# MIT-SPARK/Khronos

Hardware: AMD Instinct MI355X
Metric: active-window frames/sec (+ Mvoxel-updates/sec) at 1280x720 RGB-D+labels, 2 cm voxels (higher is better)
Workload: dtype f32

## Files before the change

### khronos_amd/csrc/khr_device.h

```cpp
#pragma once
#include <hip/hip_runtime.h>
#include <stdint.h>

namespace khr {

constexpr uint64_t kEmptyKey = ~0ull;
constexpr uint32_t kInvalidSlot = 0xffffffffu;

constexpr uint32_t BLK_UPDATED = 1u, BLK_MESH_UPDATED = 2u, BLK_TRACKING_UPDATED = 4u, BLK_HAS_ACTIVE = 8u,
                   BLK_LIVE = 16u,
                   BLK_TRACK_DIRTY = 32u,
                   BLK_ANY_KEEP = 64u,
                   BLK_HAS_NEG = 128u;
constexpr uint8_t VOX_ACTIVE = 1, VOX_EVER_FREE = 2, VOX_TO_REMOVE = 4, VOX_SEM_VALID = 8;
constexpr uint8_t VOX_OCC = 16;
constexpr uint8_t VOX_PUBLIC_MASK = 0x0f;

enum Counter : int {
  C_FREE_HEAD = 0,
  C_N_FREE,
  C_MAX_SLOT,
  C_N_VISIBLE,
  C_N_NEW,
  C_N_EF,
  C_N_LIVE,
  C_POOL_EXHAUSTED,
  C_N_UPD_LO,
  C_N_REMOVED,
  C_N_SEEDS,
  C_N_MESH,
  C_N_BAND,
  C_N_TSDF,
  C_BAND_OVERFLOW,
  C_TSDF_CURSOR,
  C_MESH_OVERFLOW,
  C_N_PROC,
  C_N_EF_A,
  C_N_PROC2,
  C_N_EF2,
  C_MP_DONE,
  C_N_ITEMS0,
  C_N_ITEMS1,
  C_N_ITEMS2,
  C_N_ITEMS3,
  C_COUNT = 32
};
enum Stat64 : int { S_UPD = 0 , S_BAND , S_MESH_VERTS, S_PRUNED, S_CUM_UPD, S_CUM_BAND, S_CUM_VISITED, S_CUM_CALLS, S_COUNT = 8 };

struct MeshDesc {
  uint32_t offset;
  uint32_t count;
};

struct DevMap {
  uint64_t* ht_keys;
  uint32_t* ht_vals;
  uint32_t ht_mask;
  uint32_t capacity;
  int4* blk_index;
  uint32_t* blk_flags;
  float* dist;
  float* weight;
  uint32_t* color;
  uint64_t* last_obs;
  ulonglong2* obs;
  uint64_t* last_occ;
  uint64_t* trk_lim;
  uint8_t* vflags;
  uint32_t* sem_label;
  float* lik;
  uint64_t* freebits;
  uint16_t* blk_band;
  uint32_t* free_slots;
  uint32_t* counters;
  unsigned long long* stats;
  MeshDesc* mesh_desc;
};

constexpr int kBandSlots = 32;
constexpr uint16_t kItemTouched = 0x8000u, kItemNeg = 0x4000u, kItemBandMask = 0x3fffu;
struct FuseList {
  uint4* a;
  uint4* b;
  uint32_t cap;
  uint32_t* counts;
};
__device__ inline uint32_t fuseClass(uint32_t band) { return band > 128u ? 0u : (band > 64u ? 1u : (band > 0u ? 2u : 3u)); }
__device__ inline uint4* fuseDescPtr(const FuseList& l, uint32_t cls, uint32_t pos) {
  uint4* const arr = cls < 2u ? l.a : l.b;
  return arr + ((cls & 1u) ? l.cap - 1u - pos : pos);
}

__host__ __device__ inline int likStride(int K) { return K <= 4 ? K : ((K + 31) & ~31); }

struct DevParams {
  float vs, vs_inv, bs, bs_inv, trunc;
  int vps, nvox, K;
  int KS;
  int with_semantics, with_tracking;
  int use_dropoff, const_weight, interp, range_mode, sem_mode;
  float dropoff_eps, max_weight, adaptive_diff, log_match, log_nomatch;
  float occ_thr;
  double temporal_buffer, temporal_window;
  int nn;
  float mesh_min_weight;
  float mesh_eps;
  int mesh_attr_source;
  int alloc_candidate;
  int rank, world;
  int dbg;
};

struct DevFrame {
  const float* depth;
  const float* range;
  const uint32_t* rgba;
  const int32_t* label;
  int32_t* dyn;
  const int32_t* obj;
  int W, H;
  float fx, fy, cx, cy, min_range, max_range;
  float R[9], t[3];
  float Rw[9], tw[3];
  uint64_t stamp;
  int has_color, has_label;
};

struct DevFrustum {
  float n[4][3];
  float infl;
  int3 bc;
  int n_steps;
  int max_steps;
  float tw[3];
};

__host__ __device__ inline uint32_t mix32(uint32_t h) {
  h ^= h >> 16;
  h *= 0x85ebca6bu;
  h ^= h >> 13;
  h *= 0xc2b2ae35u;
  h ^= h >> 16;
  return h;
}

__host__ __device__ inline int ownerOf(int x, int y, int z, int world) {
  if (world <= 1) return 0;
  const uint32_t h = mix32(static_cast<uint32_t>(x) * 73856093u ^
                           mix32(static_cast<uint32_t>(y) * 19349663u ^ mix32(static_cast<uint32_t>(z) * 83492791u)));
  return static_cast<int>((static_cast<uint64_t>(h) * static_cast<uint64_t>(world)) >> 32);
}

__host__ __device__ inline uint64_t packKey(int x, int y, int z) {
  return (static_cast<uint64_t>(static_cast<uint32_t>(x + (1 << 20)) & 0x1fffffu)) |
         (static_cast<uint64_t>(static_cast<uint32_t>(y + (1 << 20)) & 0x1fffffu) << 21) |
         (static_cast<uint64_t>(static_cast<uint32_t>(z + (1 << 20)) & 0x1fffffu) << 42);
}
__host__ __device__ inline void unpackKey(uint64_t k, int* x, int* y, int* z) {
  *x = static_cast<int>(k & 0x1fffffu) - (1 << 20);
  *y = static_cast<int>((k >> 21) & 0x1fffffu) - (1 << 20);
  *z = static_cast<int>((k >> 42) & 0x1fffffu) - (1 << 20);
}
__host__ __device__ inline uint32_t hashKey(uint64_t k) {
  return mix32(static_cast<uint32_t>(k) ^ mix32(static_cast<uint32_t>(k >> 32) + 0x9e3779b9u));
}

__device__ inline uint32_t htLookup(const DevMap& m, uint64_t key) {
  uint32_t h = hashKey(key) & m.ht_mask;
  while (true) {
    const uint64_t k = m.ht_keys[h];
    if (k == key) return m.ht_vals[h];
    if (k == kEmptyKey) return kInvalidSlot;
    h = (h + 1) & m.ht_mask;
  }
}

__device__ inline void htInsertUnique(const DevMap& m, uint64_t key, uint32_t slot) {
  uint32_t h = hashKey(key) & m.ht_mask;
  while (true) {
    const unsigned long long prev =
        atomicCAS(reinterpret_cast<unsigned long long*>(&m.ht_keys[h]), static_cast<unsigned long long>(kEmptyKey),
                  static_cast<unsigned long long>(key));
    if (prev == kEmptyKey) {
      m.ht_vals[h] = slot;
      return;
    }
    h = (h + 1) & m.ht_mask;
  }
}

__device__ inline void xform(const float* R, const float* t, float x, float y, float z, float* o) {
  o[0] = ((R[0] * x + R[1] * y) + R[2] * z) + t[0];
  o[1] = ((R[3] * x + R[4] * y) + R[5] * z) + t[1];
  o[2] = ((R[6] * x + R[7] * y) + R[8] * z) + t[2];
}

__device__ inline bool pointInFrustum(const DevFrustum& fr, const float* pc, float max_range) {
  bool in = !(pc[2] < -fr.infl);
  const float n2 = (pc[0] * pc[0] + pc[1] * pc[1]) + pc[2] * pc[2];
  const float lim = max_range + fr.infl;
  in = in && !(n2 > lim * lim);
#pragma unroll
  for (int k = 0; k < 4; ++k) {
    const float d = (pc[0] * fr.n[k][0] + pc[1] * fr.n[k][1]) + pc[2] * fr.n[k][2];
    in = in && !(d < -fr.infl);
  }
  return in;
}
__device__ inline bool blockIsCandidate(const DevParams& p, const DevFrustum& fr, const float* R, const float* t, float max_range,
                                        int bx, int by, int bz) {
  if (p.alloc_candidate == 0) {
    float pc[3];
    xform(R, t, (static_cast<float>(bx) + 0.5f) * p.bs, (static_cast<float>(by) + 0.5f) * p.bs, (static_cast<float>(bz) + 0.5f) * p.bs, pc);
    return pointInFrustum(fr, pc, max_range);
  }
  const int b[3] = {bx, by, bz}, bc[3] = {fr.bc.x, fr.bc.y, fr.bc.z};
  float cand[3][2];
  int nc[3];
#pragma unroll
  for (int a = 0; a < 3; ++a) {
    nc[a] = 0;
#pragma unroll
    for (int e = -1; e <= 1; ++e) {
      const int d = b[a] - bc[a] + e;
      if (d < -fr.max_steps || d > fr.max_steps) continue;
      const float pw = fr.tw[a] + static_cast<float>(d) * p.bs;
      if (static_cast<int>(floorf(pw * p.bs_inv)) == b[a] && nc[a] < 2) cand[a][nc[a]++] = pw;
    }
  }
  for (int i = 0; i < nc[0]; ++i)
    for (int j = 0; j < nc[1]; ++j)
      for (int k = 0; k < nc[2]; ++k) {
        float pc[3];
        xform(R, t, cand[0][i], cand[1][j], cand[2][k], pc);
        if (pointInFrustum(fr, pc, max_range)) return true;
      }
  return false;
}

constexpr uint64_t kSeedFlag = 1ull << 63;
__device__ inline uint64_t motionPixelVoxel(const DevParams& p, float r, float d, int u, int v, float fx, float fy, float cx, float cy,
                                            const float* Rw, const float* tw, float md_max_range, float min_z_world, uint64_t* block_key,
                                            int* lin_out) {
  if (!(r > 0.f && !(r > md_max_range))) return ~0ull;
  const float x = ((static_cast<float>(u) - cx) / fx) * d;
  const float y = ((static_cast<float>(v) - cy) / fy) * d;
  float pw[3];
  xform(Rw, tw, x, y, d, pw);
  if (pw[2] < min_z_world) return ~0ull;
  const int bx = static_cast<int>(floorf(pw[0] * p.bs_inv)), by = static_cast<int>(floorf(pw[1] * p.bs_inv)),
            bz = static_cast<int>(floorf(pw[2] * p.bs_inv));
  const float ox = static_cast<float>(bx) * p.bs, oy = static_cast<float>(by) * p.bs, oz = static_cast<float>(bz) * p.bs;
  const int vx = static_cast<int>(floorf((pw[0] - ox) * p.vs_inv));
  const int vy = static_cast<int>(floorf((pw[1] - oy) * p.vs_inv));
  const int vz = static_cast<int>(floorf((pw[2] - oz) * p.vs_inv));
  *block_key = packKey(bx, by, bz);
  if (!(vx >= 0 && vy >= 0 && vz >= 0 && vx < p.vps && vy < p.vps && vz < p.vps)) return ~0ull;
  *lin_out = vx + p.vps * (vy + p.vps * vz);
  return packKey(bx * p.vps + vx, by * p.vps + vy, bz * p.vps + vz);
}
__device__ inline uint64_t motionPixelKey(const DevMap& m, const DevParams& p, float r, float d, int u, int v, float fx,
                                          float fy, float cx, float cy, const float* Rw, const float* tw,
                                          float md_max_range, float min_z_world, int ignore_epoch = 0) {
  uint64_t bkey = 0ull;
  int lin = 0;
  uint64_t key = motionPixelVoxel(p, r, d, u, v, fx, fy, cx, cy, Rw, tw, md_max_range, min_z_world, &bkey, &lin);
  if (key == ~0ull) return key;
  uint32_t slot = htLookup(m, bkey);
  if (slot != kInvalidSlot && ignore_epoch != 0 && m.blk_index[slot].w == ignore_epoch) slot = kInvalidSlot;
  if (slot == kInvalidSlot) return ~0ull;
  if (m.vflags[static_cast<size_t>(slot) * p.nvox + lin] & VOX_EVER_FREE) key |= kSeedFlag;
  return key;
}

__device__ inline uint64_t lastObserved(const DevMap& m, size_t slot, uint32_t lin, int nvox) {
  const ulonglong2 w = m.obs[slot * static_cast<size_t>(nvox >> 6) + (lin >> 6)];
  return ((w.x >> (lin & 63u)) & 1ull) ? w.y : m.last_obs[slot * static_cast<size_t>(nvox) + lin];
}

__device__ inline double toSeconds(uint64_t ns) { return static_cast<double>(ns) / 1e9; }

__device__ inline uint32_t laneId() { return __lane_id(); }

__device__ inline uint32_t waveAggInc(uint32_t* counter, bool pred) {
  const unsigned long long mask = __ballot(pred);
  if (mask == 0) return 0;
  const uint32_t lane = laneId();
  const uint32_t rank = __popcll(mask & ((1ull << lane) - 1ull));
  const int leader = __ffsll(static_cast<long long>(mask)) - 1;
  uint32_t base = 0;
  if (lane == static_cast<uint32_t>(leader)) base = atomicAdd(counter, static_cast<uint32_t>(__popcll(mask)));
  base = __shfl(base, leader);
  return base + rank;
}

__device__ inline uint8_t toU8(float f) {
  float r = floorf(f + 0.5f);
  r = fminf(255.f, fmaxf(0.f, r));
  return static_cast<uint8_t>(r);
}

__device__ inline void publishSeedCount(const DevMap& m, volatile uint32_t* host_seed, uint32_t ticket) {
  host_seed[0] = atomicAdd(&m.counters[C_N_SEEDS], 0u);
  __threadfence_system();
  host_seed[1] = ticket;
  __threadfence_system();
}

constexpr int kUpdateStatSlots = 2048;

__device__ inline void beginIntegrate(DevMap m, int nvox, uint32_t* wg_stats) {
  unsigned long long u = 0, b = 0;
  uint2* __restrict__ st = reinterpret_cast<uint2*>(wg_stats);
#pragma unroll 4
  for (int i = threadIdx.x; i < kUpdateStatSlots; i += blockDim.x) {
    const uint2 v = st[i];
// ... 57 lines not shown
```

### khronos_amd/csrc/khr_kernels_fusion.h

```cpp
#pragma once
#include "khr_device.h"

namespace khr {


constexpr int kTile = 16;
constexpr int kMaxTick = 8;

__device__ inline void ingestTile(const float* __restrict__ depth_in, const uint8_t* __restrict__ rgb_in,
                                  const int32_t* __restrict__ label_in, float* __restrict__ depth, float* __restrict__ range,
                                  uint32_t* __restrict__ rgba, int32_t* __restrict__ label, int32_t* __restrict__ dyn,
                                  float* __restrict__ tile_max, int tile, int tw, int W, int H, float fx, float fy, float cx,
                                  float cy, int range_mode, float* d_out, float* r_out) {
  const int tx = tile % tw, ty = tile / tw;
  const int u = tx * kTile + (threadIdx.x & 15), v = ty * kTile + (threadIdx.x >> 4);
  float r = 0.f, d = 0.f;
  if (u < W && v < H) {
    const int i = v * W + u;
    d = depth_in[i];
    if (d > 0.f && isfinite(d)) {
      if (range_mode == 0) {
        r = d;
      } else {
        const float x = (static_cast<float>(u) - cx) / fx, y = (static_cast<float>(v) - cy) / fy;
// ... 332 lines not shown
        if (umax < -1.f || vmax < -1.f || umin > static_cast<float>(f.W) || vmin > static_cast<float>(f.H)) {
          keep = false;
        } else {
          const int tx0 = max(0, (static_cast<int>(floorf(umin)) - 1) / kTile);
          const int ty0 = max(0, (static_cast<int>(floorf(vmin)) - 1) / kTile);
          const int tx1 = min(tw - 1, (static_cast<int>(ceilf(umax)) + 2) / kTile);
          const int ty1 = min(th - 1, (static_cast<int>(ceilf(vmax)) + 2) / kTile);
          if (tx1 >= tx0 && ty1 >= ty0) {
            const int nx = tx1 - tx0 + 1, nt = nx * (ty1 - ty0 + 1);
            float mr = 0.f;
            for (int t = lane; t < nt; t += 64) mr = fmaxf(mr, tile_max[(ty0 + t / nx) * tw + tx0 + t % nx]);
#pragma unroll
            for (int o = 32; o > 0; o >>= 1) mr = fmaxf(mr, __shfl_xor(mr, o));
            if (mr < zmin - p.trunc - margin) keep = false;
          }
        }
      }
    }
    if (keep) {
      uint32_t kslot = 0;
      if (lane == 0) {
        kslot = atomicAdd(&s_nkeep, 1u);
        s_blk[kslot] = make_uint4(slot, static_cast<uint32_t>(bi.x), static_cast<uint32_t>(bi.y), static_cast<uint32_t>(bi.z));
      }
      kslot = __shfl(kslot, 0);
      const uint32_t lpi = 64u / wpb, item = lane / lpi, sub = lane % lpi;
      bool ikeep = true;
      if (tile_max && (p.dbg & 256) == 0) {
        const float margin = 1e-3f;
        const int patches = (p.vps * p.vps) >> 6, rows = 64 / p.vps, zr = p.vps / (static_cast<int>(wpb) / patches);
        const int y0 = (static_cast<int>(item) % patches) * rows, z0 = (static_cast<int>(item) / patches) * zr;
        const float lo[3] = {static_cast<float>(bi.x) * p.bs + 0.5f * p.vs, static_cast<float>(bi.y) * p.bs + (static_cast<float>(y0) + 0.5f) * p.vs,
                             static_cast<float>(bi.z) * p.bs + (static_cast<float>(z0) + 0.5f) * p.vs};
        const float ex[3] = {p.bs - p.vs, static_cast<float>(rows - 1) * p.vs, static_cast<float>(zr - 1) * p.vs};
        float zmin = 1e30f, zmax = -1e30f, umin = 1e30f, umax = -1e30f, vmin = 1e30f, vmax = -1e30f;
        float pcs[8][3];
#pragma unroll
        for (int k = 0; k < 8; ++k) {
          xform(f.R, f.t, lo[0] + ((k & 1) ? ex[0] : 0.f), lo[1] + ((k & 2) ? ex[1] : 0.f), lo[2] + ((k & 4) ? ex[2] : 0.f), pcs[k]);
          zmin = fminf(zmin, pcs[k][2]);
          zmax = fmaxf(zmax, pcs[k][2]);
        }
        if (zmax <= -margin) ikeep = false;
        if (zmin > f.max_range + margin) ikeep = false;
        if (p.range_mode == 0 && zmax < f.min_range - margin) ikeep = false;
        if (ikeep && zmin > 0.05f) {
#pragma unroll
          for (int k = 0; k < 8; ++k) {
            const float iz = __builtin_amdgcn_rcpf(pcs[k][2]);
            const float u = (pcs[k][0] * f.fx) * iz + f.cx, v = (pcs[k][1] * f.fy) * iz + f.cy;
            umin = fminf(umin, u); umax = fmaxf(umax, u);
            vmin = fminf(vmin, v); vmax = fmaxf(vmax, v);
          }
          if (umax < -2.f || vmax < -2.f || umin > static_cast<float>(f.W) + 1.f || vmin > static_cast<float>(f.H) + 1.f) {
            ikeep = false;
          } else {
            const int tx0 = max(0, (static_cast<int>(floorf(umin)) - 2) / kTile);
            const int ty0 = max(0, (static_cast<int>(floorf(vmin)) - 2) / kTile);
            const int tx1 = min(tw - 1, (static_cast<int>(ceilf(umax)) + 3) / kTile);
            const int ty1 = min(th - 1, (static_cast<int>(ceilf(vmax)) + 3) / kTile);
            const int nx = tx1 - tx0 + 1, nt = nx * (ty1 - ty0 + 1);
            if (tx1 >= tx0 && ty1 >= ty0 && nt <= 16 * static_cast<int>(lpi)) {
              float m0 = 0.f, m1 = 0.f;
              int t = static_cast<int>(sub);
              for (; t + static_cast<int>(lpi) < nt; t += 2 * static_cast<int>(lpi)) {
                const int t2 = t + static_cast<int>(lpi);
                const float a = tile_max[(ty0 + t / nx) * tw + tx0 + t % nx];
                const float b = tile_max[(ty0 + t2 / nx) * tw + tx0 + t2 % nx];
                m0 = fmaxf(m0, a);
                m1 = fmaxf(m1, b);
              }
              if (t < nt) m0 = fmaxf(m0, tile_max[(ty0 + t / nx) * tw + tx0 + t % nx]);
              float mr = fmaxf(m0, m1);
              for (uint32_t o = 1; o < lpi; o <<= 1) mr = fmaxf(mr, __shfl_xor(mr, static_cast<int>(o)));
              if (mr < zmin - p.trunc - margin) ikeep = false;
            }
          }
        }
      }
      if (ikeep && sub == 0 && item_mask) {
        const size_t mi = static_cast<size_t>(slot) * wpb + item;
        const uint32_t sh = 8u * static_cast<uint32_t>(mi & 3);
        const uint32_t old = atomicOr(&item_mask[mi >> 2], (1u << cam) << sh);
        if ((old >> sh) & 0xffu) ikeep = false;
      }
      if (ikeep && sub == 0) {
        const uint32_t cls = fuseClass(m.blk_band[static_cast<size_t>(slot) * kBandSlots + item] & kItemBandMask);
        s_item[cls][atomicAdd(&s_ccnt[cls], 1u)] = static_cast<uint16_t>((kslot << 8) | item);
      }
    }
  }
  __syncthreads();
  if (threadIdx.x < 4) s_off[threadIdx.x] = s_ccnt[threadIdx.x] ? atomicAdd(&out.counts[threadIdx.x], s_ccnt[threadIdx.x]) : 0u;
  if (threadIdx.x == 0 && s_nkeep) atomicAdd(n_tsdf, s_nkeep);
  __syncthreads();
#pragma unroll
  for (uint32_t cls = 0; cls < 4; ++cls) {
    for (uint32_t i = threadIdx.x; i < s_ccnt[cls]; i += blockDim.x) {
      const uint32_t it = s_item[cls][i];
      uint4 d = s_blk[it >> 8];
      d.x |= (it & 0xffu) << 24;
      *fuseDescPtr(out, cls, s_off[cls] + i) = d;
    }
  }
  __syncthreads();
  }
}

__global__ __launch_bounds__(256) void k_cull_blocks(DevMap m, DevParams p, DevFrame f,
                                                    const uint32_t* __restrict__ work, FuseList out, uint32_t wpb,
                                                    const float* __restrict__ tile_max, int tw, int th) {
  cullBlocks(m, p, f, work, &m.counters[C_N_VISIBLE], out, wpb, &m.counters[C_N_TSDF], tile_max, tw, th, blockIdx.x, gridDim.x);
}

struct TickFrames {
  DevFrame f[kMaxTick];
  const float* tile_max[kMaxTick];
};
__global__ __launch_bounds__(256) void k_tick_cull(DevMap m, DevParams p, TickFrames t, const uint32_t* __restrict__ work,
                                                  uint32_t list_stride, uint4* __restrict__ desc, uint32_t desc_stride, uint32_t wpb,
                                                  uint32_t* __restrict__ tick_counts, int use_tiles, int tw, int th,
                                                  uint32_t* __restrict__ item_mask) {
  const int cam = blockIdx.y;
  const int lc = item_mask ? 0 : cam;
  FuseList out{desc + static_cast<size_t>(2 * lc) * desc_stride, desc + static_cast<size_t>(2 * lc + 1) * desc_stride, desc_stride,
               &tick_counts[2 * kMaxTick + 4 * lc]};
  cullBlocks(m, p, t.f[cam], work + static_cast<size_t>(cam) * list_stride, &tick_counts[2 * cam], out, wpb, &tick_counts[2 * cam + 1],
             use_tiles ? t.tile_max[cam] : nullptr, tw, th, blockIdx.x, gridDim.x, item_mask, static_cast<uint32_t>(cam));
}

__global__ __launch_bounds__(256) void k_alloc_list(DevMap m, const int* __restrict__ idx, int n,
                                                   uint32_t* __restrict__ new_list) {
  const int i = blockIdx.x * blockDim.x + threadIdx.x;
  bool need = false;
  int bx = 0, by = 0, bz = 0;
  if (i < n) {
    bx = idx[3 * i];
    by = idx[3 * i + 1];
    bz = idx[3 * i + 2];
    need = htLookup(m, packKey(bx, by, bz)) == kInvalidSlot;
  }
  const uint32_t fidx = waveAggInc(&m.counters[C_FREE_HEAD], need);
  bool got = false;
  uint32_t slot = kInvalidSlot;
  if (need) {
    if (fidx < m.counters[C_N_FREE]) {
      slot = m.free_slots[fidx];
      got = true;
      m.blk_index[slot] = make_int4(bx, by, bz, 0);
      m.blk_flags[slot] = BLK_LIVE | BLK_TRACK_DIRTY | BLK_ANY_KEEP;
      m.mesh_desc[slot] = MeshDesc{0u, 0u};
      htInsertUnique(m, packKey(bx, by, bz), slot);
      atomicMax(&m.counters[C_MAX_SLOT], slot + 1);
    } else {
      atomicAdd(&m.counters[C_POOL_EXHAUSTED], 1u);
    }
  }
  const uint32_t nidx = waveAggInc(&m.counters[C_N_NEW], got);
  if (got) new_list[nidx] = slot;
}

__global__ __launch_bounds__(256) void k_list_live(DevMap m, uint32_t* __restrict__ work, uint32_t* counter,
                                                  uint32_t require_flags, FuseList out = FuseList{nullptr, nullptr, 0u, nullptr},
                                                  uint32_t wpb = 0u) {
  const uint32_t s = blockIdx.x * blockDim.x + threadIdx.x;
  bool live = false;
  if (s < m.counters[C_MAX_SLOT]) {
    const uint32_t fl = m.blk_flags[s];
    live = (fl & BLK_LIVE) && ((fl & require_flags) == require_flags);
  }
  const uint32_t idx = waveAggInc(counter, live);
  if (live) work[idx] = s;
  if (out.a) {
    const unsigned long long mask = __ballot(live);
    if (mask) {
      const uint32_t lane = laneId();
      const int leader = __ffsll(static_cast<long long>(mask)) - 1;
      uint32_t base = 0;
      if (lane == static_cast<uint32_t>(leader)) base = atomicAdd(&out.counts[3], static_cast<uint32_t>(__popcll(mask)) * wpb);
      base = __shfl(base, leader) + static_cast<uint32_t>(__popcll(mask & ((1ull << lane) - 1ull))) * wpb;
      if (live) {
        const int4 bi = m.blk_index[s];
        for (uint32_t it = 0; it < wpb; ++it)
          *fuseDescPtr(out, 3u, base + it) =
              make_uint4(s | (it << 24), static_cast<uint32_t>(bi.x), static_cast<uint32_t>(bi.y), static_cast<uint32_t>(bi.z));
      }
    }
  }
}

__device__ inline void initBlock(const DevMap& m, const DevParams& p, size_t slot) {
  const int nv = p.nvox;
  {
    const uint4 z = make_uint4(0, 0, 0, 0);
    uint4* d4 = reinterpret_cast<uint4*>(m.dist + slot * nv);
    uint4* w4 = reinterpret_cast<uint4*>(m.weight + slot * nv);
    uint4* c4 = reinterpret_cast<uint4*>(m.color + slot * nv);
    uint4* l4 = reinterpret_cast<uint4*>(m.sem_label + slot * nv);
    for (int i = threadIdx.x; i < nv / 4; i += blockDim.x) {
      d4[i] = z;
      w4[i] = z;
      c4[i] = z;
      if (p.with_semantics) l4[i] = z;
    }
    uint4* f4 = reinterpret_cast<uint4*>(m.vflags + slot * nv);
    for (int i = threadIdx.x; i < nv / 16; i += blockDim.x) f4[i] = z;
    if (threadIdx.x < kBandSlots) m.blk_band[slot * kBandSlots + threadIdx.x] = 0;
    if (p.with_tracking) {
      uint4* o4 = reinterpret_cast<uint4*>(m.last_obs + slot * nv);
      uint4* q4 = reinterpret_cast<uint4*>(m.last_occ + slot * nv);
      for (int i = threadIdx.x; i < nv / 2; i += blockDim.x) {
        o4[i] = z;
        q4[i] = z;
      }
      uint64_t* fb = m.freebits + slot * (nv / 64);
      for (int i = threadIdx.x; i < nv / 64; i += blockDim.x) {
        fb[i] = 0ull;
        m.obs[slot * (nv / 64) + i] = make_ulonglong2(0ull, 0ull);
      }
    }
  }
}

__device__ inline void initBlocks(const DevMap& m, const DevParams& p, const uint32_t* __restrict__ new_list, uint32_t bid,
                                  uint32_t nblk) {
  const uint32_t n = m.counters[C_N_NEW];
  for (uint32_t b = bid; b < n; b += nblk) initBlock(m, p, new_list[b]);
}

struct BoxSetupZero {
  uint32_t* w;
  uint32_t n;
};
__global__ __launch_bounds__(256) void k_setup_box(DevMap m, DevParams p, int3 lo, int3 dim, uint32_t n,
                                                  uint32_t* __restrict__ work, FuseList out, uint32_t wpb, uint32_t* wg_stats,
                                                  BoxSetupZero zero) {
  const uint32_t b = blockIdx.x;
  if (b >= n) return;
  if (b == 0) {
    beginIntegrate(m, p.nvox, wg_stats);
    if (threadIdx.x == 0) {
      m.counters[C_FREE_HEAD] = n;
      m.counters[C_MAX_SLOT] = n;
      m.counters[C_N_VISIBLE] = n;
      out.counts[3] = n * wpb;
    }
    if (zero.w != nullptr && threadIdx.x < zero.n) zero.w[threadIdx.x] = 0u;
  }
  const int bx = lo.x + static_cast<int>(b / static_cast<uint32_t>(dim.y * dim.z));
  const int by = lo.y + static_cast<int>((b / static_cast<uint32_t>(dim.z)) % static_cast<uint32_t>(dim.y));
  const int bz = lo.z + static_cast<int>(b % static_cast<uint32_t>(dim.z));
  if (threadIdx.x == 0) {
    m.blk_index[b] = make_int4(bx, by, bz, 0);
    m.blk_flags[b] = BLK_LIVE | BLK_TRACK_DIRTY | BLK_ANY_KEEP;
    m.mesh_desc[b] = MeshDesc{0u, 0u};
    htInsertUnique(m, packKey(bx, by, bz), b);
    work[b] = b;
  }
  if (threadIdx.x < wpb)
    *fuseDescPtr(out, 3u, b * wpb + threadIdx.x) =
        make_uint4(b | (threadIdx.x << 24), static_cast<uint32_t>(bx), static_cast<uint32_t>(by), static_cast<uint32_t>(bz));
  initBlock(m, p, b);
}

__global__ __launch_bounds__(256) void k_init_blocks(DevMap m, DevParams p, const uint32_t* __restrict__ new_list) {
  initBlocks(m, p, new_list, blockIdx.x, gridDim.x);
}

__global__ __launch_bounds__(256) void k_init_cull(DevMap m, DevParams p, DevFrame f, const uint32_t* __restrict__ new_list,
                                                  const uint32_t* __restrict__ work, FuseList out, uint32_t wpb,
                                                  const float* __restrict__ tile_max, int tw, int th, uint32_t n_cull) {
  if (blockIdx.x < n_cull)
    cullBlocks(m, p, f, work, &m.counters[C_N_VISIBLE], out, wpb, &m.counters[C_N_TSDF], tile_max, tw, th, blockIdx.x, n_cull);
  else
    initBlocks(m, p, new_list, blockIdx.x - n_cull, gridDim.x - n_cull);
}

__device__ inline uint32_t foldItemRecords(uint32_t* __restrict__ blk_flags, uint16_t* __restrict__ blk_band, uint32_t s) {
  static_assert(kBandSlots == 32, "record row = 4 x 16 bytes");
  uint4* const row = reinterpret_cast<uint4*>(blk_band + static_cast<size_t>(s) * kBandSlots);
  uint32_t any = 0u;
  uint4 r[4];
#pragma unroll
  for (int i = 0; i < 4; ++i) {
    r[i] = row[i];
    any |= r[i].x | r[i].y | r[i].z | r[i].w;
  }
  const uint32_t tm = static_cast<uint32_t>(kItemTouched) * 0x00010001u, nm = static_cast<uint32_t>(kItemNeg) * 0x00010001u;
  uint32_t fl = blk_flags[s];
  if ((any & tm) == 0u) return fl;
  fl |= BLK_UPDATED | BLK_MESH_UPDATED | BLK_TRACKING_UPDATED | ((any & nm) ? BLK_HAS_NEG : 0u);
  blk_flags[s] = fl;
  const uint32_t keep = static_cast<uint32_t>(kItemBandMask) * 0x00010001u;
#pragma unroll
  for (int i = 0; i < 4; ++i) row[i] = make_uint4(r[i].x & keep, r[i].y & keep, r[i].z & keep, r[i].w & keep);
  return fl;
}
__global__ __launch_bounds__(256) void k_tracking_select(DevMap m, uint64_t lim_active, uint64_t lim_free, int force_full,
                                                        uint32_t* __restrict__ proc, uint32_t* __restrict__ ef_list,
                                                        uint32_t* __restrict__ cnt ,
                                                        uint32_t* __restrict__ cnt_next, uint16_t* __restrict__ fold_band) {
  const uint32_t s = blockIdx.x * blockDim.x + threadIdx.x;
  if (s == 0) { cnt_next[0] = 0u; cnt_next[1] = 0u; }
  bool need = false, touched = false, reload = false;
  if (s < m.counters[C_MAX_SLOT]) {
    const uint32_t fl = fold_band ? foldItemRecords(m.blk_flags, fold_band, s) : m.blk_flags[s];
    if (fl & BLK_LIVE) {
      touched = fl & BLK_TRACKING_UPDATED;
      need = force_full || (fl & (BLK_TRACKING_UPDATED | BLK_TRACK_DIRTY));
      reload = need;
      if (!need) {
        const ulonglong2 lim = reinterpret_cast<const ulonglong2*>(m.trk_lim)[s];
        need = !(lim_active <= lim.x && lim_free <= lim.y);
      }
    }
  }
  const uint32_t ip = waveAggInc(&cnt[0], need);
  if (need) {
    proc[ip] = s | (reload ? 0x80000000u : 0u);
    reinterpret_cast<ulonglong2*>(m.trk_lim)[s] = make_ulonglong2(~0ull, ~0ull);
    m.blk_flags[s] = m.blk_flags[s] & ~(BLK_TRACKING_UPDATED | BLK_HAS_ACTIVE | BLK_TRACK_DIRTY | BLK_ANY_KEEP);
  }
  const uint32_t ie = waveAggInc(&cnt[1], touched);
  if (touched) ef_list[ie] = s;
}

template <int VPS, int CH>
__global__ __launch_bounds__(256) void k_tracking_update(DevMap m, DevParams p, uint64_t stamp, uint64_t prev_stamp,
                                                        uint64_t lim_active, uint64_t lim_free,
                                                        const uint32_t* __restrict__ proc, const uint32_t* __restrict__ n_proc) {
  constexpr int NV = VPS * VPS * VPS;
  __shared__ uint64_t s_min[2][4];
  __shared__ uint32_t s_bits;
  const uint32_t n = *n_proc * CH;
  for (uint32_t wi = blockIdx.x; wi < n; wi += gridDim.x) {
    const uint32_t pe = proc[wi / CH];
    const uint32_t s = pe & 0x7fffffffu;
    const bool reload = (pe >> 31) != 0u;
    const int g0 = static_cast<int>(wi % CH) * (NV / 4 / CH);
    const size_t slot = s;
    const float4* __restrict__ dist4 = reinterpret_cast<const float4*>(m.dist + slot * NV);
    const ulonglong2* __restrict__ lobs2 = reinterpret_cast<const ulonglong2*>(m.last_obs + slot * NV);
    uint64_t* __restrict__ locc = m.last_occ + slot * NV;
    uint32_t* __restrict__ vfl4 = reinterpret_cast<uint32_t*>(m.vflags + slot * NV);
    uint64_t* __restrict__ fb = m.freebits + slot * (NV / 64);
    bool any_active = false, any_keep = false;
    uint64_t a_min = ~0ull, f_min = ~0ull;
    if (threadIdx.x == 0) s_bits = 0u;
    constexpr int G = NV / 4 / CH / 256 > 0 ? NV / 4 / CH / 256 : 1;
    constexpr int GEND = NV / 4 / CH;
    float4 d_[G];
    ulonglong2 oa_[G], ob_[G], ca_[G], cb_[G], ow_[G];
    uint32_t v4_[G];
    uint32_t need_[G];
#pragma unroll
    for (int q = 0; q < G; ++q) {
      const int gl = threadIdx.x + 256 * q, g = g0 + gl;
      if (gl < GEND) {
        d_[q] = reload ? dist4[g] : make_float4(0.f, 0.f, 0.f, 0.f);
        ow_[q] = m.obs[slot * (NV / 64) + (g >> 4)];
        v4_[q] = vfl4[g];
      }
    }
#pragma unroll
    for (int q = 0; q < G; ++q) {
      const int gl = threadIdx.x + 256 * q, g = g0 + gl;
      need_[q] = 0u;
      ca_[q] = make_ulonglong2(0ull, 0ull);
      cb_[q] = ca_[q];
      oa_[q] = ca_[q];
      ob_[q] = ca_[q];
      if (gl < GEND) {
        const uint32_t b4 = static_cast<uint32_t>(ow_[q].x >> ((4u * static_cast<uint32_t>(g)) & 63u)) & 0xfu;
        if ((b4 & 3u) != 3u) oa_[q] = lobs2[2 * g];
        if ((b4 & 12u) != 12u) ob_[q] = lobs2[2 * g + 1];
        const float dd[4] = {d_[q].x, d_[q].y, d_[q].z, d_[q].w};
#pragma unroll
        for (int k = 0; k < 4; ++k) {
          const uint8_t v = static_cast<uint8_t>(v4_[q] >> (8 * k));
          const bool occ_k = reload ? (dd[k] < p.occ_thr) : ((v & VOX_OCC) != 0);
          if (!occ_k && !(v & VOX_OCC) && !(v & VOX_EVER_FREE)) need_[q] |= 1u << k;
        }
        if (need_[q] & 3u) ca_[q] = reinterpret_cast<const ulonglong2*>(locc)[2 * g];
        if (need_[q] & 12u) cb_[q] = reinterpret_cast<const ulonglong2*>(locc)[2 * g + 1];
      }
    }
#pragma unroll
    for (int q = 0; q < G; ++q) {
      const int gl = threadIdx.x + 256 * q, g = g0 + gl;
      if (gl >= GEND) continue;
      const uint32_t v4 = v4_[q];
      const float dd[4] = {d_[q].x, d_[q].y, d_[q].z, d_[q].w};
      uint64_t lo[4] = {oa_[q].x, oa_[q].y, ob_[q].x, ob_[q].y};
      {
        const uint32_t b4 = static_cast<uint32_t>(ow_[q].x >> ((4u * static_cast<uint32_t>(g)) & 63u)) & 0xfu;
#pragma unroll
        for (int k = 0; k < 4; ++k)
          if ((b4 >> k) & 1u) lo[k] = ow_[q].y;
      }
      const uint64_t stored[4] = {ca_[q].x, ca_[q].y, cb_[q].x, cb_[q].y};
      uint32_t nv4 = 0, freebits4 = 0;
#pragma unroll
      for (int k = 0; k < 4; ++k) {
        const uint8_t v = static_cast<uint8_t>(v4 >> (8 * k));
        const bool was_occ = v & VOX_OCC;
        const bool occ = reload ? (dd[k] < p.occ_thr) : was_occ;
        uint64_t oc = stored[k];
        if (occ) {
          oc = stamp;
        } else if (was_occ) {
          oc = prev_stamp;
          locc[4 * g + k] = prev_stamp;
        }
        const bool was_active = v & VOX_ACTIVE;
        const bool active = lo[k] >= lim_active;
        uint8_t nv = static_cast<uint8_t>((v & ~(VOX_ACTIVE | VOX_OCC)) | (active ? VOX_ACTIVE : 0) | (occ ? VOX_OCC : 0));
        if (was_active && !active) nv |= VOX_TO_REMOVE;
        any_active |= active;
        any_keep |= !(nv & VOX_TO_REMOVE);
        if (active) a_min = lo[k] < a_min ? lo[k] : a_min;
        const bool ever = nv & VOX_EVER_FREE;
        const bool is_free = !ever && (oc < lim_free) && (lo[k] != 0ull);
        if (ever || is_free) freebits4 |= 1u << k;
        if (!occ && !ever && !is_free && lo[k] != 0ull) f_min = oc < f_min ? oc : f_min;
        nv4 |= static_cast<uint32_t>(nv) << (8 * k);
      }
      if (nv4 != v4) vfl4[g] = nv4;
      uint64_t w = static_cast<uint64_t>(freebits4) << (4 * (threadIdx.x & 15));
#pragma unroll
      for (int o = 1; o < 16; o <<= 1) {
        const uint32_t lo32 = __shfl_xor(static_cast<uint32_t>(w), o);
        const uint32_t hi32 = __shfl_xor(static_cast<uint32_t>(w >> 32), o);
        w |= (static_cast<uint64_t>(hi32) << 32) | lo32;
      }
      if ((threadIdx.x & 15) == 0) fb[g >> 4] = w;
    }
#pragma unroll
    for (int o = 32; o > 0; o >>= 1) {
      const uint64_t a2 = (static_cast<uint64_t>(__shfl_xor(static_cast<uint32_t>(a_min >> 32), o)) << 32) |
                          __shfl_xor(static_cast<uint32_t>(a_min), o);
      const uint64_t f2 = (static_cast<uint64_t>(__shfl_xor(static_cast<uint32_t>(f_min >> 32), o)) << 32) |
                          __shfl_xor(static_cast<uint32_t>(f_min), o);
      a_min = a2 < a_min ? a2 : a_min;
      f_min = f2 < f_min ? f2 : f_min;
    }
    __syncthreads();
    const uint32_t wbits = (__builtin_amdgcn_ballot_w64(any_active) != 0ull ? 1u : 0u) | (__builtin_amdgcn_ballot_w64(any_keep) != 0ull ? 2u : 0u);
    if ((threadIdx.x & 63) == 0) {
      s_min[0][threadIdx.x >> 6] = a_min;
      s_min[1][threadIdx.x >> 6] = f_min;
      if (wbits) atomicOr(&s_bits, wbits);
    }
    __syncthreads();
    if (threadIdx.x == 0) {
      const uint32_t bits = s_bits;
      uint64_t a = s_min[0][0], f = s_min[1][0];
#pragma unroll
      for (int w = 1; w < 4; ++w) {
        a = s_min[0][w] < a ? s_min[0][w] : a;
        f = s_min[1][w] < f ? s_min[1][w] : f;
      }
      unsigned long long* lim = reinterpret_cast<unsigned long long*>(m.trk_lim) + 2 * static_cast<size_t>(s);
      if (a != ~0ull) atomicMin(&lim[0], static_cast<unsigned long long>(a));
      if (f != ~0ull) atomicMin(&lim[1], static_cast<unsigned long long>(f));
      if (bits) atomicOr(&m.blk_flags[s], ((bits & 1u) ? BLK_HAS_ACTIVE : 0u) | ((bits & 2u) ? BLK_ANY_KEEP : 0u));
    }
    __syncthreads();
  }
}

__constant__ int8_t c_nbr26[26][3] = {
    {-1, 0, 0}, {1, 0, 0}, {0, -1, 0}, {0, 1, 0}, {0, 0, -1}, {0, 0, 1},
    {-1, -1, 0}, {-1, 1, 0}, {1, -1, 0}, {1, 1, 0}, {-1, 0, -1}, {-1, 0, 1}, {1, 0, -1}, {1, 0, 1},
    {0, -1, -1}, {0, -1, 1}, {0, 1, -1}, {0, 1, 1},
    {-1, -1, -1}, {-1, -1, 1}, {-1, 1, -1}, {-1, 1, 1}, {1, -1, -1}, {1, -1, 1}, {1, 1, -1}, {1, 1, 1}};

constexpr int kHaloRecWords = 66;

struct RemoteHalo {
  const uint64_t* recs;
  const uint64_t* ht_keys;
  const uint32_t* ht_vals;
  uint32_t ht_mask;
};

template <int VPS>
__global__ __launch_bounds__(256) void k_ever_free(DevMap m, DevParams p, const uint32_t* __restrict__ ef_list,
                                                  const uint32_t* __restrict__ ef_count, RemoteHalo rh) {
  constexpr int NV = VPS * VPS * VPS;
  constexpr int NW = NV / 64;
  constexpr int T = VPS + 2;
  __shared__ uint32_t s_row[T * T];
  __shared__ uint64_t s_bits[27][NW];
  __shared__ const uint64_t* s_src[27];
  const uint32_t n = *ef_count;
  for (uint32_t b = blockIdx.x; b < n; b += gridDim.x) {
    const size_t slot = ef_list[b];
    const int4 bi = m.blk_index[slot];
    __syncthreads();
    if (threadIdx.x < 27) {
      const int dx = threadIdx.x % 3 - 1, dy = (threadIdx.x / 3) % 3 - 1, dz = threadIdx.x / 9 - 1;
      const uint64_t key = packKey(bi.x + dx, bi.y + dy, bi.z + dz);
      const uint32_t ns = (threadIdx.x == 13) ? static_cast<uint32_t>(slot) : htLookup(m, key);
      const uint64_t* src = nullptr;
      if (ns != kInvalidSlot) {
        src = m.freebits + static_cast<size_t>(ns) * NW;
      } else if (rh.recs) {
        uint32_t h = hashKey(key) & rh.ht_mask;
        while (true) {
          const uint64_t k = rh.ht_keys[h];
          if (k == key) {
            src = rh.recs + static_cast<size_t>(rh.ht_vals[h]) * kHaloRecWords + 2;
            break;
          }
          if (k == kEmptyKey) break;
          h = (h + 1) & rh.ht_mask;
        }
      }
      s_src[threadIdx.x] = src;
    }
    __syncthreads();
    for (int i = threadIdx.x; i < 27 * NW; i += 256) {
      const uint64_t* src = s_src[i / NW];
      s_bits[i / NW][i % NW] = src ? src[i % NW] : 0ull;
    }
    __syncthreads();
    for (int r = threadIdx.x; r < T * T; r += 256) {
      const int ty = r % T, tz = r / T;
      int y = ty - 1, z = tz - 1, sy = 1, sz = 1;
      if (y < 0) { y += VPS; sy = 0; } else if (y >= VPS) { y -= VPS; sy = 2; }
      if (z < 0) { z += VPS; sz = 0; } else if (z >= VPS) { z -= VPS; sz = 2; }
      const int lin0 = VPS * (y + VPS * z);
      const uint32_t mid = static_cast<uint32_t>((s_bits[1 + 3 * sy + 9 * sz][lin0 >> 6] >> (lin0 & 63)) & ((1u << VPS) - 1u));
      const uint32_t left = static_cast<uint32_t>((s_bits[0 + 3 * sy + 9 * sz][(lin0 + VPS - 1) >> 6] >> ((lin0 + VPS - 1) & 63)) & 1u);
      const uint32_t right = static_cast<uint32_t>((s_bits[2 + 3 * sy + 9 * sz][lin0 >> 6] >> (lin0 & 63)) & 1u);
      s_row[r] = left | (mid << 1) | (right << (VPS + 1));
    }
    __syncthreads();
    uint8_t* __restrict__ vfl = m.vflags + slot * NV;
    for (int r = threadIdx.x; r < VPS * VPS; r += 256) {
      const int iy = r % VPS, iz = r / VPS;
      const int c = (iy + 1) + T * (iz + 1);
      const uint32_t self = s_row[c];
      uint32_t ok = self & (self >> 1) & (self << 1);
      const uint32_t f1[4] = {s_row[c - 1], s_row[c + 1], s_row[c - T], s_row[c + T]};
#pragma unroll
      for (int k = 0; k < 4; ++k) {
        ok &= f1[k];
        if (p.nn >= 18) ok &= (f1[k] >> 1) & (f1[k] << 1);
      }
      if (p.nn >= 18) {
        const uint32_t f2[4] = {s_row[c - 1 - T], s_row[c + 1 - T], s_row[c - 1 + T], s_row[c + 1 + T]};
#pragma unroll
        for (int k = 0; k < 4; ++k) {
          ok &= f2[k];
          if (p.nn == 26) ok &= (f2[k] >> 1) & (f2[k] << 1);
        }
      }
      uint32_t cand = (ok >> 1) & ((1u << VPS) - 1u);
      const int base = VPS * (iy + VPS * iz);
      while (cand) {
        const int x = __ffs(cand) - 1;
        cand &= cand - 1u;
        const uint8_t v = vfl[base + x];
        if (!(v & VOX_EVER_FREE)) vfl[base + x] = v | VOX_EVER_FREE;
      }
    }
  }
}

__global__ void k_live_bound(DevMap m, int64_t* __restrict__ out, int n_out, int index) {
  const uint32_t n_free = m.counters[C_N_FREE], head = min(m.counters[C_FREE_HEAD], n_free);
  const int64_t live = static_cast<int64_t>(m.capacity) - static_cast<int64_t>(n_free - head);
  for (int i = threadIdx.x; i < n_out; i += blockDim.x) out[i] = i == index ? live : 0;
}

template <int VPS>
__global__ __launch_bounds__(256) void k_export_halo(DevMap m, const uint32_t* __restrict__ list,
                                                    const uint32_t* __restrict__ n_list, uint64_t* __restrict__ recs,
                                                    uint32_t cap) {
  constexpr int NW = VPS * VPS * VPS / 64;
  const uint32_t n = min(*n_list, cap);
  if (blockIdx.x == 0 && threadIdx.x == 0 && *n_list > cap) atomicAdd(&m.counters[C_POOL_EXHAUSTED], 1u);
  const uint32_t total = cap * kHaloRecWords;
  for (uint32_t i = blockIdx.x * blockDim.x + threadIdx.x; i < total; i += gridDim.x * blockDim.x) {
    const uint32_t r = i / kHaloRecWords, w = i % kHaloRecWords;
    uint64_t v = 0ull;
    if (r < n) {
      const uint32_t slot = list[r];
      if (w == 0) {
        const int4 bi = m.blk_index[slot];
        v = packKey(bi.x, bi.y, bi.z);
      } else if (w == 1) {
        v = 1ull;
      } else if (w - 2 < NW) {
        v = m.freebits[static_cast<size_t>(slot) * NW + (w - 2)];
      }
    }
    recs[i] = v;
  }
}

__global__ __launch_bounds__(256) void k_import_halo(const uint64_t* __restrict__ recs, uint32_t n_total, int rank,
                                                    int world, uint64_t* __restrict__ ht_keys,
                                                    uint32_t* __restrict__ ht_vals, uint32_t ht_mask) {
  const uint32_t r = blockIdx.x * blockDim.x + threadIdx.x;
  if (r >= n_total) return;
  if (recs[static_cast<size_t>(r) * kHaloRecWords + 1] != 1ull) return;
  const uint64_t key = recs[static_cast<size_t>(r) * kHaloRecWords];
  int x, y, z;
  unpackKey(key, &x, &y, &z);
  if (ownerOf(x, y, z, world) == rank) return;
  uint32_t h = hashKey(key) & ht_mask;
  while (true) {
    const unsigned long long prev = atomicCAS(reinterpret_cast<unsigned long long*>(&ht_keys[h]),
                                              static_cast<unsigned long long>(kEmptyKey), static_cast<unsigned long long>(key));
    if (prev == kEmptyKey) {
      ht_vals[h] = r;
      return;
    }
    h = (h + 1) & ht_mask;
  }
}

}
```

Baseline: 4285.

## Skip redundant last-obs/last-occ loads and ever-free blocks without free candidates

Tracking update now marks trusted blocks and uses the previous freebits word to infer, per voxel, whether last_obs and last_occ must be read. Voxels already known free or settled skip those 64-bit loads, which cuts memory traffic in quiet blocks. The kernel also records a per-block BLK_EF_CAND flag when any voxel is a free candidate, so k_ever_free can skip blocks with none and avoid the 27-neighbour lookup. This depends on freebits staying consistent with the stamps, so it risks subtle correctness drift.

```diff
diff --git a/khronos_amd/csrc/khr_device.h b/khronos_amd/csrc/khr_device.h
--- a/khronos_amd/csrc/khr_device.h
+++ b/khronos_amd/csrc/khr_device.h
@@ -11,7 +11,8 @@
                    BLK_LIVE = 16u,
                    BLK_TRACK_DIRTY = 32u,
                    BLK_ANY_KEEP = 64u,
-                   BLK_HAS_NEG = 128u;
+                   BLK_HAS_NEG = 128u,
+                   BLK_EF_CAND = 256u;
 constexpr uint8_t VOX_ACTIVE = 1, VOX_EVER_FREE = 2, VOX_TO_REMOVE = 4, VOX_SEM_VALID = 8;
 constexpr uint8_t VOX_OCC = 16;
 constexpr uint8_t VOX_PUBLIC_MASK = 0x0f;
diff --git a/khronos_amd/csrc/khr_kernels_fusion.h b/khronos_amd/csrc/khr_kernels_fusion.h
--- a/khronos_amd/csrc/khr_kernels_fusion.h
+++ b/khronos_amd/csrc/khr_kernels_fusion.h
@@ -658,13 +658,14 @@
                                                         uint32_t* __restrict__ cnt_next, uint16_t* __restrict__ fold_band) {
   const uint32_t s = blockIdx.x * blockDim.x + threadIdx.x;
   if (s == 0) { cnt_next[0] = 0u; cnt_next[1] = 0u; }
-  bool need = false, touched = false, reload = false;
+  bool need = false, touched = false, reload = false, trusted = false;
   if (s < m.counters[C_MAX_SLOT]) {
     const uint32_t fl = fold_band ? foldItemRecords(m.blk_flags, fold_band, s) : m.blk_flags[s];
     if (fl & BLK_LIVE) {
       touched = fl & BLK_TRACKING_UPDATED;
       need = force_full || (fl & (BLK_TRACKING_UPDATED | BLK_TRACK_DIRTY));
       reload = need;
+      trusted = !force_full && !(fl & BLK_TRACK_DIRTY);
       if (!need) {
         const ulonglong2 lim = reinterpret_cast<const ulonglong2*>(m.trk_lim)[s];
         need = !(lim_active <= lim.x && lim_free <= lim.y);
@@ -673,9 +674,9 @@
   }
   const uint32_t ip = waveAggInc(&cnt[0], need);
   if (need) {
-    proc[ip] = s | (reload ? 0x80000000u : 0u);
+    proc[ip] = s | (reload ? 0x80000000u : 0u) | (trusted ? 0x40000000u : 0u);
     reinterpret_cast<ulonglong2*>(m.trk_lim)[s] = make_ulonglong2(~0ull, ~0ull);
-    m.blk_flags[s] = m.blk_flags[s] & ~(BLK_TRACKING_UPDATED | BLK_HAS_ACTIVE | BLK_TRACK_DIRTY | BLK_ANY_KEEP);
+    m.blk_flags[s] = m.blk_flags[s] & ~(BLK_TRACKING_UPDATED | BLK_HAS_ACTIVE | BLK_TRACK_DIRTY | BLK_ANY_KEEP | BLK_EF_CAND);
   }
   const uint32_t ie = waveAggInc(&cnt[1], touched);
   if (touched) ef_list[ie] = s;
@@ -689,10 +690,13 @@
   __shared__ uint64_t s_min[2][4];
   __shared__ uint32_t s_bits;
   const uint32_t n = *n_proc * CH;
+  const bool occ_not_free = stamp >= lim_free;
   for (uint32_t wi = blockIdx.x; wi < n; wi += gridDim.x) {
     const uint32_t pe = proc[wi / CH];
-    const uint32_t s = pe & 0x7fffffffu;
+    const uint32_t s = pe & 0x3fffffffu;
     const bool reload = (pe >> 31) != 0u;
+    const bool trusted = ((pe >> 30) & 1u) != 0u;
+    const bool quiet = trusted && !reload;
     const int g0 = static_cast<int>(wi % CH) * (NV / 4 / CH);
     const size_t slot = s;
     const float4* __restrict__ dist4 = reinterpret_cast<const float4*>(m.dist + slot * NV);
@@ -700,7 +704,7 @@
     uint64_t* __restrict__ locc = m.last_occ + slot * NV;
     uint32_t* __restrict__ vfl4 = reinterpret_cast<uint32_t*>(m.vflags + slot * NV);
     uint64_t* __restrict__ fb = m.freebits + slot * (NV / 64);
-    bool any_active = false, any_keep = false;
+    bool any_active = false, any_keep = false, any_cand = false;
     uint64_t a_min = ~0ull, f_min = ~0ull;
     if (threadIdx.x == 0) s_bits = 0u;
     constexpr int G = NV / 4 / CH / 256 > 0 ? NV / 4 / CH / 256 : 1;
@@ -709,34 +713,49 @@
     ulonglong2 oa_[G], ob_[G], ca_[G], cb_[G], ow_[G];
     uint32_t v4_[G];
     uint32_t need_[G];
+    uint32_t skip_[G];
+    uint64_t pf_[G];
 #pragma unroll
     for (int q = 0; q < G; ++q) {
       const int gl = threadIdx.x + 256 * q, g = g0 + gl;
+      pf_[q] = 0ull;
       if (gl < GEND) {
         d_[q] = reload ? dist4[g] : make_float4(0.f, 0.f, 0.f, 0.f);
         ow_[q] = m.obs[slot * (NV / 64) + (g >> 4)];
         v4_[q] = vfl4[g];
+        if (trusted) pf_[q] = fb[g >> 4];
       }
     }
 #pragma unroll
     for (int q = 0; q < G; ++q) {
       const int gl = threadIdx.x + 256 * q, g = g0 + gl;
       need_[q] = 0u;
+      skip_[q] = 0u;
       ca_[q] = make_ulonglong2(0ull, 0ull);
       cb_[q] = ca_[q];
       oa_[q] = ca_[q];
       ob_[q] = ca_[q];
       if (gl < GEND) {
         const uint32_t b4 = static_cast<uint32_t>(ow_[q].x >> ((4u * static_cast<uint32_t>(g)) & 63u)) & 0xfu;
-        if ((b4 & 3u) != 3u) oa_[q] = lobs2[2 * g];
-        if ((b4 & 12u) != 12u) ob_[q] = lobs2[2 * g + 1];
+        const uint32_t pf4 = static_cast<uint32_t>(pf_[q] >> ((4u * static_cast<uint32_t>(g)) & 63u)) & 0xfu;
+        uint32_t need_lo = 0u;
         const float dd[4] = {d_[q].x, d_[q].y, d_[q].z, d_[q].w};
 #pragma unroll
         for (int k = 0; k < 4; ++k) {
           const uint8_t v = static_cast<uint8_t>(v4_[q] >> (8 * k));
           const bool occ_k = reload ? (dd[k] < p.occ_thr) : ((v & VOX_OCC) != 0);
-          if (!occ_k && !(v & VOX_OCC) && !(v & VOX_EVER_FREE)) need_[q] |= 1u << k;
+          const bool ever_k = (v & VOX_EVER_FREE) != 0;
+          const bool prevfree = ((pf4 >> k) & 1u) != 0u;
+          if (!occ_k && !(v & VOX_OCC) && !ever_k) {
+            if (prevfree) skip_[q] |= 16u << k; else need_[q] |= 1u << k;
+          }
+          const bool open_k = !ever_k && (occ_k ? !occ_not_free : !prevfree);
+          if (!quiet || (v & VOX_ACTIVE) || open_k) need_lo |= 1u << k;
         }
+        need_lo &= ~b4;
+        skip_[q] |= ~(need_lo | b4) & 0xfu;
+        if (need_lo & 3u) oa_[q] = lobs2[2 * g];
+        if (need_lo & 12u) ob_[q] = lobs2[2 * g + 1];
         if (need_[q] & 3u) ca_[q] = reinterpret_cast<const ulonglong2*>(locc)[2 * g];
         if (need_[q] & 12u) cb_[q] = reinterpret_cast<const ulonglong2*>(locc)[2 * g + 1];
       }
@@ -769,16 +788,19 @@
           locc[4 * g + k] = prev_stamp;
         }
         const bool was_active = v & VOX_ACTIVE;
-        const bool active = lo[k] >= lim_active;
+        const bool lo_out = (skip_[q] >> k) & 1u, oc_out = (skip_[q] >> (4 + k)) & 1u;
+        const bool active = !lo_out && lo[k] >= lim_active;
+        const bool seen = lo_out || lo[k] != 0ull;
         uint8_t nv = static_cast<uint8_t>((v & ~(VOX_ACTIVE | VOX_OCC)) | (active ? VOX_ACTIVE : 0) | (occ ? VOX_OCC : 0));
         if (was_active && !active) nv |= VOX_TO_REMOVE;
         any_active |= active;
         any_keep |= !(nv & VOX_TO_REMOVE);
         if (active) a_min = lo[k] < a_min ? lo[k] : a_min;
         const bool ever = nv & VOX_EVER_FREE;
-        const bool is_free = !ever && (oc < lim_free) && (lo[k] != 0ull);
+        const bool is_free = !ever && (oc_out || oc < lim_free) && seen;
+        any_cand |= is_free;
         if (ever || is_free) freebits4 |= 1u << k;
-        if (!occ && !ever && !is_free && lo[k] != 0ull) f_min = oc < f_min ? oc : f_min;
+        if (!occ && !ever && !is_free && seen) f_min = oc < f_min ? oc : f_min;
         nv4 |= static_cast<uint32_t>(nv) << (8 * k);
       }
       if (nv4 != v4) vfl4[g] = nv4;
@@ -801,7 +823,8 @@
       f_min = f2 < f_min ? f2 : f_min;
     }
     __syncthreads();
-    const uint32_t wbits = (__builtin_amdgcn_ballot_w64(any_active) != 0ull ? 1u : 0u) | (__builtin_amdgcn_ballot_w64(any_keep) != 0ull ? 2u : 0u);
+    const uint32_t wbits = (__builtin_amdgcn_ballot_w64(any_active) != 0ull ? 1u : 0u) | (__builtin_amdgcn_ballot_w64(any_keep) != 0ull ? 2u : 0u) |
+                           (__builtin_amdgcn_ballot_w64(any_cand) != 0ull ? 4u : 0u);
     if ((threadIdx.x & 63) == 0) {
       s_min[0][threadIdx.x >> 6] = a_min;
       s_min[1][threadIdx.x >> 6] = f_min;
@@ -819,7 +842,7 @@
       unsigned long long* lim = reinterpret_cast<unsigned long long*>(m.trk_lim) + 2 * static_cast<size_t>(s);
       if (a != ~0ull) atomicMin(&lim[0], static_cast<unsigned long long>(a));
       if (f != ~0ull) atomicMin(&lim[1], static_cast<unsigned long long>(f));
-      if (bits) atomicOr(&m.blk_flags[s], ((bits & 1u) ? BLK_HAS_ACTIVE : 0u) | ((bits & 2u) ? BLK_ANY_KEEP : 0u));
+      if (bits) atomicOr(&m.blk_flags[s], ((bits & 1u) ? BLK_HAS_ACTIVE : 0u) | ((bits & 2u) ? BLK_ANY_KEEP : 0u) | ((bits & 4u) ? BLK_EF_CAND : 0u));
     }
     __syncthreads();
   }
@@ -852,6 +875,7 @@
   const uint32_t n = *ef_count;
   for (uint32_t b = blockIdx.x; b < n; b += gridDim.x) {
     const size_t slot = ef_list[b];
+    if (!(m.blk_flags[slot] & BLK_EF_CAND)) continue;
     const int4 bi = m.blk_index[slot];
     __syncthreads();
     if (threadIdx.x < 27) {
```

Measured after the change: 4235. 0.988x the previous value.
